# cvjena/mvlm

Hardware: AMD Instinct MI355X
Metric: views/sec (render+CNN+fuse) per mesh, 256x256x96 views (higher is better)
Workload: dtype f32; 1 GPU; configs[2] BU_3DFE-RGB+depth.json: 96 views @ 256x256 of one 99458-triangle textured synthetic face OBJ, 84 landmarks, 4 input channels (RGB+depth), seeded random weights; views_total=96, views_per_gpu=96, landmarks=84, in_channels=4, triangles=99458, selection_method=simple, parallelism=1 GPU, no collective

## Files before the change

mvlm_amd/csrc/conv_kernel.h:

```cpp
#ifndef MVLM_CONV_KERNEL_H
#define MVLM_CONV_KERNEL_H
#include <cstdlib>
#include <string>
#include <type_traits>

#include "common.h"

using f32x16 = __attribute__((ext_vector_type(16))) float;
using f32x4 = __attribute__((ext_vector_type(4))) float;

namespace {

constexpr unsigned INVALID_OFF = 0xFFFFFFFFu;

template <int I, int N, class F>
__device__ __forceinline__ void static_for(F&& f) {
    if constexpr (I < N) {
        f(std::integral_constant<int, I>{});
        static_for<I + 1, N>(f);
    }
}

template <int COUT_T_, int TW_, int TRI_, int NIMG_, int KS_, int CK_, bool SPLITK_ = false>
struct Cfg {
// ... 372 lines not shown
    const int e = tid + i * 256;
    return (e < C::WJOBS ? e : e - C::WJOBS) / ((C::TRI / 2) * C::PW);
}

template <class C>
__device__ __forceinline__ void wino_mask_tail(const ConvArgs& a, int cb, int tid, WinoStage<C>& ws) {
#pragma unroll
    for (int i = 0; i < C::X_ITERS; ++i) {
        const bool okc = cb + wino_job_channel<C>(tid, i) < a.cin;
#pragma unroll
        for (int q = 0; q < 3; ++q) ws.msk[i][q] = okc ? ws.msk[i][q] : 0u;
#pragma unroll
        for (int q = 0; q < 4; ++q) ws.off[i][q] = okc ? ws.off[i][q] : 0u;
    }
}

template <class C>
__device__ __forceinline__ void wino_main(const ConvArgs& a, float* smem, const int tid, const int y0, const int x0, const int b0,
                                          const int co0, const unsigned HWin, const int woff, f32x16 (&acc)[C::MT][C::NT], long long* t_loop) {
    static_assert(!C::WINO || (C::WT / 4) % 256 == 0, "every lane owns whole float4s of the weight slice");
    static_assert(!C::WINO || 256 * C::X_ITERS - C::WJOBS <= C::WJOBS, "a lane without a job repeats an earlier job");
    static_assert(!C::WINO || C::TRI % 2 == 0, "rows 2p and 2p + 1 of a tile share one mask: a tile is whole row pairs of an image whose height is a multiple of it");
    const int lane = tid & 63, wave = tid >> 6, half = lane >> 5, l31 = lane & 31;
    WinoStage<C> ws;
    constexpr int JPC = (C::TRI / 2) * C::PW;
#pragma unroll
    for (int i = 0; i < C::X_ITERS; ++i) {
        const int e0 = tid + i * 256;
        const int e = e0 < C::WJOBS ? e0 : e0 - C::WJOBS;
        const int c = e / JPC;
        const int rem = e - c * JPC;
        const int p = rem / C::PW;
        const int xx = rem - p * C::PW;
        const int y = y0 + 2 * p - 1, x = x0 + xx - 1;
        const bool okx = x >= 0 && x < a.W && b0 < a.B;
#pragma unroll
        for (int q = 0; q < 4; ++q) {
            const bool ok = okx && y + q >= 0 && y + q < a.H;
            ws.msk[i][q == 0 ? 0 : q == 3 ? 2 : 1] = ok ? 0xFFFFFFFFu : 0u;
            ws.off[i][q] = ok ? (unsigned(c) * HWin + unsigned((y + q) * a.W + x)) * 4u : 0u;
        }
        ws.lds[i] = c * C::PLANE + (p * C::PW + xx) * 4;
        ws.bn[i] = c;
    }
    {
        const int row = tid / (C::COUT_T / 4);
        const int c4 = tid - row * (C::COUT_T / 4);
        const int tap = row / C::CK;
        const int c = row - tap * C::CK;
        ws.woff = unsigned((tap * a.cin_pad + c) * a.cout_pad + co0 + c4 * 4) * 4u;
    }
    constexpr int TAPS_STEP = 256 / ((C::COUT_T / 4) * C::CK);
    static_assert(!C::WINO || 256 % ((C::COUT_T / 4) * C::CK) == 0, "256 float4s of the weight slice are whole taps");
    const size_t w_step = size_t(TAPS_STEP) * a.cin_pad * a.cout_pad * 4;
    ws.floor = __int_as_float(__builtin_amdgcn_readfirstlane(a.pre_scale != nullptr ? 0 : int(0xFF800000u)));
#pragma unroll
    for (int m = 0; m < C::MT; ++m) {
        ws.abase[m] = woff + m * 32;
        wino_opaque(ws.abase[m]);
    }
#pragma unroll
    for (int s = 0; s < 2; ++s)
#pragma unroll
        for (int cp = 0; cp < C::CK / 2; ++cp) {
            ws.bbase[s][cp] = s * C::STAGE + (2 * cp + half) * C::PLANE + (wave * C::WP * C::PW + l31) * 4;
            wino_opaque(ws.bbase[s][cp]);
        }
    float* const sbn = smem + 2 * C::STAGE;
    const char* const in0 = reinterpret_cast<const char*>(a.in + size_t((b0 < a.B ? b0 : 0) * a.in_ctot + a.in_coff) * HWin);
    const char* const w0 = reinterpret_cast<const char*>(a.w);
    constexpr int T_TOT = C::X_ITERS + C::W_ITERS;
    const int last = a.cin_pad - C::CK;
    const bool odd = (a.cin_pad / C::CK) & 1;
    if (last == 0) wino_mask_tail<C>(a, 0, tid, ws);
    static_for<0, T_TOT>([&](auto tc) { issue_item_wino<C, decltype(tc)::value>(in0, w0, w_step, ws); });
    for (int i = tid; i < a.cin_pad; i += 256) {
        sbn[2 * i] = a.pre_scale != nullptr ? a.pre_scale[i] : 1.f;
        sbn[2 * i + 1] = a.pre_scale != nullptr ? a.pre_shift[i] : -0.f;
    }
    __syncthreads();
    static_for<0, T_TOT>([&](auto tc) { bn_item_wino<C, decltype(tc)::value>(sbn, 0, ws); });
    if (odd) {
        static_for<0, T_TOT>([&](auto tc) { write_item_wino<C, decltype(tc)::value, 1>(smem, tid, ws); });
    } else {
        static_for<0, T_TOT>([&](auto tc) { write_item_wino<C, decltype(tc)::value, 0>(smem, tid, ws); });
    }
    __syncthreads();
#if defined(MVLM_CONV_TIMING)
    *t_loop = clock64();
#endif
    f32x16 wacc[C::MT][4 * C::WP];
#pragma unroll
    for (int m = 0; m < C::MT; ++m)
#pragma unroll
        for (int q = 0; q < 4 * C::WP; ++q) wacc[m][q] = f32x16{0.f, 0.f, 0.f, 0.f, 0.f, 0.f, 0.f, 0.f, 0.f, 0.f, 0.f, 0.f, 0.f, 0.f, 0.f, 0.f};
    if (last > 0) {
        int cb = 0;
        const size_t in_step = size_t(C::CK) * HWin * 4, w_cstep = size_t(C::CK) * a.cout_pad * 4;
        const char* in_nx = in0 + in_step;
        const char* w_nx = w0 + w_cstep;
        if (odd) {
            compute_chunk_wino<C, 1, true>(smem, sbn, in_nx, w_nx, w_step, C::CK, tid, ws, wacc);
            __syncthreads();
            cb = C::CK, in_nx += in_step, w_nx += w_cstep;
        }
        wino_forget_bases<C>(ws);
        for (; cb + C::CK < last; cb += 2 * C::CK) {
            compute_chunk_wino<C, 0, true>(smem, sbn, in_nx, w_nx, w_step, cb + C::CK, tid, ws, wacc);
            __syncthreads();
            in_nx += in_step, w_nx += w_cstep;
            compute_chunk_wino<C, 1, true>(smem, sbn, in_nx, w_nx, w_step, cb + 2 * C::CK, tid, ws, wacc);
            __syncthreads();
            in_nx += in_step, w_nx += w_cstep;
        }
        wino_forget_bases<C>(ws);
        wino_mask_tail<C>(a, last, tid, ws);
        compute_chunk_wino<C, 0, true>(smem, sbn, in_nx, w_nx, w_step, last, tid, ws, wacc);
        __syncthreads();
    }
    compute_chunk_wino<C, 1, false>(smem, sbn, nullptr, nullptr, 0, 0, tid, ws, wacc);
    static_for<0, C::MT>([&](auto mc) {
        constexpr int m = decltype(mc)::value;
        static_for<0, C::WP>([&](auto pc) {
            constexpr int p = decltype(pc)::value;
#pragma unroll
            for (int r = 0; r < 16; ++r) {
                const float m0 = wacc[m][4 * p][r], m1 = wacc[m][4 * p + 1][r], m2 = wacc[m][4 * p + 2][r], m3 = wacc[m][4 * p + 3][r];
                acc[m][2 * p][r] = (m0 + m1) + m2;
                acc[m][2 * p + 1][r] = (m1 - m2) - m3;
            }
        });
    });
    (void)t_loop;
}

template <class C>
struct Wino4Stage {
    static constexpr int N = C::WINO4 ? C::X_ITERS : 1;
    static constexpr int NW = C::WINO4 ? C::W_ITERS : 1;
    unsigned off[N][6];
    unsigned msk[N][3];
    int lds4[N], lds2[N];
    int bn[N];
    unsigned woff[NW];
    int wlds[NW];
    float xw[N][6];
    float bn_s[N], bn_t[N];
    f32x4 wv[NW];
    float floor;
    int abase;
    int bbase4[2][C::CK / 2], bbase2[2][C::CK / 2];
};

template <class C, int T>
__device__ __forceinline__ void issue_item_wino4(const char* in_cb, const char* w_cb, Wino4Stage<C>& ws) {
    if constexpr (T < C::X_ITERS) {
#pragma unroll
        for (int r = 0; r < 6; ++r) {
            wino_opaque(ws.off[T][r]);
            ws.xw[T][r] = *reinterpret_cast<const float*>(in_cb + ws.off[T][r]);
        }
    } else {
        constexpr int I = T - C::X_ITERS;
        wino_opaque(ws.woff[I]);
        ws.wv[I] = *reinterpret_cast<const f32x4*>(w_cb + ws.woff[I]);
    }
}

template <class C, int T>
__device__ __forceinline__ void bn_item_wino4(const float* sbn, int cb, Wino4Stage<C>& ws) {
    if constexpr (T < C::X_ITERS) {
        const float2 st = *reinterpret_cast<const float2*>(sbn + 2 * (cb + ws.bn[T]));
        ws.bn_s[T] = st.x;
        ws.bn_t[T] = st.y;
    }
}

template <class C, int T, int NEXT>
__device__ __forceinline__ void write_item_wino4(float* smem, const Wino4Stage<C>& ws) {
    if constexpr (T < C::X_ITERS) {
        float d[6];
#pragma unroll
        for (int r = 0; r < 6; ++r) {
            const float v = fmaxf(fmaf(ws.xw[T][r], ws.bn_s[T], ws.bn_t[T]), ws.floor);
            d[r] = __uint_as_float(__float_as_uint(v) & ws.msk[T][r == 0 ? 0 : r == 5 ? 2 : 1]);
        }
        const float v0 = fmaf(-1.5f, d[3], fmaf(-2.f, d[2], fmaf(1.5f, d[1], d[0]))) + d[4];
        const float v1 = fmaf(-0.5f, d[3], fmaf(-2.5f, d[2], -d[1])) + d[4];
        const float v2 = fmaf(-2.5f, d[3], fmaf(0.5f, d[2], d[1])) + d[4];
        const float v3 = fmaf(0.5f, d[3], fmaf(-0.5f, d[1], -d[2])) + d[4];
        const float v4 = fmaf(-2.f, d[3], fmaf(2.f, d[1], -d[2])) + d[4];
        const float v5 = fmaf(-1.5f, d[4], fmaf(-2.f, d[3], fmaf(1.5f, d[2], d[1]))) + d[5];
        *reinterpret_cast<f32x4*>(smem + NEXT * C::STAGE + ws.lds4[T]) = f32x4{v0, v1, v2, v3};
        *reinterpret_cast<float2*>(smem + NEXT * C::STAGE + ws.lds2[T]) = make_float2(v4, v5);
    } else {
        constexpr int I = T - C::X_ITERS;
        reinterpret_cast<f32x4*>(smem + NEXT * C::STAGE + C::XT_PAD)[ws.wlds[I]] = ws.wv[I];
    }
}

template <class C, int CUR, bool STAGE_NEXT>
__device__ __forceinline__ void compute_chunk_wino4(float* smem, const float* sbn, const char* in_cb, const char* w_cb, int cb_next,
                                                    Wino4Stage<C>& ws, f32x16 (&acc)[6]) {
    constexpr int T_TOT = C::X_ITERS + C::W_ITERS;
    constexpr int ISSUE_SPAN = C::KSTEPS / 2 > 0 ? C::KSTEPS / 2 : 1;
    constexpr int WRITE_SPAN = ISSUE_SPAN;
    constexpr int WRITE_START = C::KSTEPS - WRITE_SPAN;
    const float* const st = smem + CUR * C::STAGE;
    float av[2][6];
    f32x4 bv4[2];
    float2 bv2[2];
#pragma unroll
    for (int t = 0; t < 6; ++t) av[0][t] = st[ws.abase + t * 3 * C::CK * C::COUT_T];
    bv4[0] = *reinterpret_cast<const f32x4*>(smem + ws.bbase4[CUR][0]);
    bv2[0] = *reinterpret_cast<const float2*>(smem + ws.bbase2[CUR][0]);
    static_for<0, C::KSTEPS>([&](auto ksc) {
        constexpr int ks = decltype(ksc)::value;
        constexpr int nx = ks + 1;
        __builtin_amdgcn_s_waitcnt(0xC07F);
        __builtin_amdgcn_sched_barrier(0);
        if constexpr (nx < C::KSTEPS) {
            constexpr int kx = nx / (C::CK / 2), cp = nx % (C::CK / 2);
#pragma unroll
            for (int t = 0; t < 6; ++t) av[nx & 1][t] = st[ws.abase + ((t * 3 + kx) * C::CK + 2 * cp) * C::COUT_T];
            bv4[nx & 1] = *reinterpret_cast<const f32x4*>(smem + ws.bbase4[CUR][cp] + kx * 4);
            bv2[nx & 1] = *reinterpret_cast<const float2*>(smem + ws.bbase2[CUR][cp] + kx * 2);
        }
        auto bval = [&](auto tc) {
            constexpr int t = decltype(tc)::value;
            if constexpr (t < 4) return bv4[ks & 1][t];
            else if constexpr (t == 4) return bv2[ks & 1].x;
            else return bv2[ks & 1].y;
        };
        constexpr int LEAD = 2;
        static_for<0, 6>([&](auto tc) {
            constexpr int t = decltype(tc)::value;
            if constexpr (t < LEAD) acc[t] = __builtin_amdgcn_mfma_f32_32x32x2f32(av[ks & 1][t], bval(tc), acc[t], 0, 0, 0);
        });
        __builtin_amdgcn_sched_barrier(0);
        if constexpr (STAGE_NEXT) {
            if constexpr (ks >= WRITE_START) {
                constexpr int t_last = ((ks - WRITE_START + 1) * T_TOT + WRITE_SPAN - 1) / WRITE_SPAN - 1;
                static_assert(WRITE_START + (t_last * WRITE_SPAN) / T_TOT == ks && (t_last + 1 == T_TOT || WRITE_START + ((t_last + 1) * WRITE_SPAN) / T_TOT > ks));
                constexpr int later = (t_last + 1 < C::X_ITERS ? 6 * (C::X_ITERS - t_last - 1) + C::W_ITERS : T_TOT - t_last - 1);
                static_assert(later < 16);
                __builtin_amdgcn_s_waitcnt(0x0F70 | later);
                __builtin_amdgcn_sched_barrier(0);
            }
            static_for<0, T_TOT>([&](auto tc) {
                constexpr int t = decltype(tc)::value;
                if constexpr ((t * ISSUE_SPAN) / T_TOT == ks) {
                    issue_item_wino4<C, t>(in_cb, w_cb, ws);
                    bn_item_wino4<C, t>(sbn, cb_next, ws);
                }
                if constexpr (WRITE_START + (t * WRITE_SPAN) / T_TOT == ks) write_item_wino4<C, t, CUR ^ 1>(smem, ws);
            });
            __builtin_amdgcn_sched_barrier(0);
        }
        __builtin_amdgcn_s_setprio(1);
        static_for<0, 6>([&](auto tc) {
            constexpr int t = decltype(tc)::value;
            if constexpr (t >= LEAD) acc[t] = __builtin_amdgcn_mfma_f32_32x32x2f32(av[ks & 1][t], bval(tc), acc[t], 0, 0, 0);
        });
        __builtin_amdgcn_s_setprio(0);
        __builtin_amdgcn_sched_barrier(0);
    });
}

template <class C>
__device__ __forceinline__ void wino4_forget_bases(Wino4Stage<C>& ws) {
    wino_opaque(ws.abase);
#pragma unroll
    for (int s = 0; s < 2; ++s)
#pragma unroll
        for (int cp = 0; cp < C::CK / 2; ++cp) {
            wino_opaque(ws.bbase4[s][cp]);
            wino_opaque(ws.bbase2[s][cp]);
        }
#pragma unroll
    for (int i = 0; i < C::X_ITERS; ++i) {
        wino_opaque(ws.lds4[i]);
        wino_opaque(ws.lds2[i]);
    }
}

template <class C>
__device__ __forceinline__ int wino4_job_channel(int tid, int i) {
    const int e = tid + i * 256;
    return (e < C::WJOBS ? e : e - C::WJOBS) / ((C::TRI / 4) * C::PW);
}

template <class C>
__device__ __forceinline__ void wino4_mask_tail(const ConvArgs& a, int cb, int tid, Wino4Stage<C>& ws) {
#pragma unroll
    for (int i = 0; i < C::X_ITERS; ++i) {
        const bool okc = cb + wino4_job_channel<C>(tid, i) < a.cin;
#pragma unroll
        for (int q = 0; q < 3; ++q) ws.msk[i][q] = okc ? ws.msk[i][q] : 0u;
#pragma unroll
        for (int r = 0; r < 6; ++r) ws.off[i][r] = okc ? ws.off[i][r] : 0u;
    }
}

template <class C>
__device__ __forceinline__ void wino4_main(const ConvArgs& a, float* smem, const int tid, const int y0, const int x0, const int b0,
                                           const int co0, const unsigned HWin, const int woff, f32x16 (&acc)[C::EMT][C::ENT], long long* t_loop) {
    static_assert(!C::WINO4 || 256 * C::X_ITERS - C::WJOBS <= C::WJOBS, "a lane without a job repeats an earlier job");
    static_assert(!C::WINO4 || (C::TRI % 4 == 0 && C::ENT == 4 && C::EMT == 1), "one row quad per wave; rows 4q .. 4q + 3 of a tile share one mask");
    static_assert(!C::WINO4 || (C::WT / 4 > 256 * (C::W_ITERS - 1) && C::WT / 4 >= 256), "a lane without a float4 repeats its previous one");
    const int lane = tid & 63, wave = tid >> 6, half = lane >> 5, l31 = lane & 31;
    const int wq = C::WIDE4 ? (wave & 1) : wave;
    const int wh = C::WIDE4 ? (wave >> 1) : 0;
    Wino4Stage<C> ws;
    constexpr int JPC = (C::TRI / 4) * C::PW;
    constexpr int Q4 = JPC * 4;
#pragma unroll
    for (int i = 0; i < C::X_ITERS; ++i) {
        const int e0 = tid + i * 256;
        const int e = e0 < C::WJOBS ? e0 : e0 - C::WJOBS;
        const int c = e / JPC;
        const int rem = e - c * JPC;
        const int q = rem / C::PW;
        const int xx = rem - q * C::PW;
        const int y = y0 + 4 * q - 1, x = x0 + xx - 1;
        const bool okx = x >= 0 && x < a.W && b0 < a.B;
#pragma unroll
        for (int r = 0; r < 6; ++r) {
            const bool ok = okx && y + r >= 0 && y + r < a.H;
            if (r == 0 || r == 1 || r == 5) ws.msk[i][r == 0 ? 0 : r == 5 ? 2 : 1] = ok ? 0xFFFFFFFFu : 0u;
            ws.off[i][r] = ok ? (unsigned(c) * HWin + unsigned((y + r) * a.W + x)) * 4u : 0u;
        }
        ws.lds4[i] = c * C::PLANE + rem * 4;
        ws.lds2[i] = c * C::PLANE + Q4 + rem * 2;
        ws.bn[i] = c;
    }
#pragma unroll
    for (int i = 0; i < C::W_ITERS; ++i) {
        const int f0 = tid + i * 256;
        const int f = f0 < C::WT / 4 ? f0 : f0 - 256;
        const int row = f / (C::COUT_T / 4);
        const int c4 = f - row * (C::COUT_T / 4);
        const int tap = row / C::CK;
        const int c = row - tap * C::CK;
        ws.woff[i] = unsigned((tap * a.cin_pad + c) * a.cout_pad + co0 + c4 * 4) * 4u;
        ws.wlds[i] = f;
    }
    ws.floor = __int_as_float(__builtin_amdgcn_readfirstlane(a.pre_scale != nullptr ? 0 : int(0xFF800000u)));
    ws.abase = woff + 32 * wh;
    wino_opaque(ws.abase);
#pragma unroll
    for (int s = 0; s < 2; ++s)
#pragma unroll
        for (int cp = 0; cp < C::CK / 2; ++cp) {
            ws.bbase4[s][cp] = s * C::STAGE + (2 * cp + half) * C::PLANE + (wq * C::PW + l31) * 4;
            ws.bbase2[s][cp] = s * C::STAGE + (2 * cp + half) * C::PLANE + Q4 + (wq * C::PW + l31) * 2;
            wino_opaque(ws.bbase4[s][cp]);
            wino_opaque(ws.bbase2[s][cp]);
        }
    float* const sbn = smem + 2 * C::STAGE;
    const char* const in0 = reinterpret_cast<const char*>(a.in + size_t((b0 < a.B ? b0 : 0) * a.in_ctot + a.in_coff) * HWin);
    const char* const w0 = reinterpret_cast<const char*>(a.w);
    constexpr int T_TOT = C::X_ITERS + C::W_ITERS;
    const int last = a.cin_pad - C::CK;
    const bool odd = (a.cin_pad / C::CK) & 1;
    if (last == 0) wino4_mask_tail<C>(a, 0, tid, ws);
    static_for<0, T_TOT>([&](auto tc) { issue_item_wino4<C, decltype(tc)::value>(in0, w0, ws); });
    for (int i = tid; i < a.cin_pad; i += 256) {
        sbn[2 * i] = a.pre_scale != nullptr ? a.pre_scale[i] : 1.f;
        sbn[2 * i + 1] = a.pre_scale != nullptr ? a.pre_shift[i] : -0.f;
    }
    __syncthreads();
    static_for<0, T_TOT>([&](auto tc) { bn_item_wino4<C, decltype(tc)::value>(sbn, 0, ws); });
    if (odd) {
        static_for<0, T_TOT>([&](auto tc) { write_item_wino4<C, decltype(tc)::value, 1>(smem, ws); });
    } else {
        static_for<0, T_TOT>([&](auto tc) { write_item_wino4<C, decltype(tc)::value, 0>(smem, ws); });
    }
    __syncthreads();
#if defined(MVLM_CONV_TIMING)
    *t_loop = clock64();
#endif
    f32x16 wacc[6];
#pragma unroll
    for (int t = 0; t < 6; ++t) wacc[t] = f32x16{0.f, 0.f, 0.f, 0.f, 0.f, 0.f, 0.f, 0.f, 0.f, 0.f, 0.f, 0.f, 0.f, 0.f, 0.f, 0.f};
    if (last > 0) {
        int cb = 0;
        const size_t in_step = size_t(C::CK) * HWin * 4, w_cstep = size_t(C::CK) * a.cout_pad * 4;
        const char* in_nx = in0 + in_step;
        const char* w_nx = w0 + w_cstep;
        if (odd) {
            compute_chunk_wino4<C, 1, true>(smem, sbn, in_nx, w_nx, C::CK, ws, wacc);
            __syncthreads();
            cb = C::CK, in_nx += in_step, w_nx += w_cstep;
        }
        wino4_forget_bases<C>(ws);
        for (; cb + C::CK < last; cb += 2 * C::CK) {
            compute_chunk_wino4<C, 0, true>(smem, sbn, in_nx, w_nx, cb + C::CK, ws, wacc);
            __syncthreads();
            in_nx += in_step, w_nx += w_cstep;
            compute_chunk_wino4<C, 1, true>(smem, sbn, in_nx, w_nx, cb + 2 * C::CK, ws, wacc);
            __syncthreads();
            in_nx += in_step, w_nx += w_cstep;
        }
        wino4_forget_bases<C>(ws);
        wino4_mask_tail<C>(a, last, tid, ws);
        compute_chunk_wino4<C, 0, true>(smem, sbn, in_nx, w_nx, last, ws, wacc);
        __syncthreads();
    }
    compute_chunk_wino4<C, 1, false>(smem, sbn, nullptr, nullptr, 0, ws, wacc);
#pragma unroll
    for (int r = 0; r < 16; ++r) {
        const float m0 = wacc[0][r], m1 = wacc[1][r], m2 = wacc[2][r], m3 = wacc[3][r], m4 = wacc[4][r], m5 = wacc[5][r];
        const float s = m1 + m2, d = m1 - m2;
        acc[0][0][r] = (m0 + s) + (m3 + m4);
        acc[0][1][r] = d + fmaf(-0.5f, m4, 2.f * m3);
        acc[0][2][r] = s + fmaf(0.25f, m4, 4.f * m3);
        acc[0][3][r] = (d + fmaf(-0.125f, m4, 8.f * m3)) + m5;
    }
    (void)t_loop;
}

template <class C, bool AMAX, bool IN2 = false>
__device__ __forceinline__ void conv_tile(const ConvArgs& a_in, const int tiles_x, const int tiles_y, const int cout_tiles,
                                          const int bid, const int nblk) {
    extern __shared__ __attribute__((aligned(16))) float smem[];

    const int tid = threadIdx.x;
    const int lane = tid & 63;
    const int wave = tid >> 6;
    const int half = lane >> 5;
    const int l31 = lane & 31;

    int lid;
    {
        const int q = nblk >> 3, r = nblk & 7, xcd = bid & 7;
        lid = (xcd < r ? xcd * (q + 1) : r * (q + 1) + (xcd - r) * q) + (bid >> 3);
    }
    ConvArgs a_par;
    if constexpr (C::KS == 2) {
        a_par = a_in;
        if (a_in.n_par == 4) {
            const int pl = lid & 3;
            lid >>= 2;
            a_par.sub_y = pl >> 1;
            a_par.sub_x = pl & 1;
            a_par.w = a_in.w_par[pl];
            a_par.amax_part0 = a_in.amax_part0 + pl * a_in.amax_par_stride;
        }
    }
    const ConvArgs& a = C::KS == 2 ? a_par : a_in;
    int kp = 0;
    if constexpr (C::SPLITK) {
        if (a.kparts > 1) {
            kp = lid % a.kparts;
            lid /= a.kparts;
        }
    }
    const int tile_id = lid;
    const int ct = lid % cout_tiles;
    const int pt = lid / cout_tiles;
    const int tx = pt % tiles_x;
    const int ty = (pt / tiles_x) % tiles_y;
    const int tb = pt / (tiles_x * tiles_y);
    const int x0 = tx * C::TW, y0 = ty * C::TRI, b0 = tb * C::NIMG, co0 = ct * C::COUT_T;

#if defined(MVLM_CONV_TIMING)
    const long long t_start = clock64();
    long long t_loop = t_start;
#endif
    const int H = a.H, W = a.W;
    const int Hin = a.up_in ? (H >> 1) : H, Win = a.up_in ? (W >> 1) : W;
    const unsigned HWin = unsigned(Hin) * unsigned(Win);

    unsigned goff[C::X_ITERS];
    unsigned goff2[C::X_ITERS];
#pragma unroll
    for (int i = 0; i < C::X_ITERS; ++i) {
        const int e = tid + i * 256;
        const int c = e / C::PLANE;
        const int rem = e - c * C::PLANE;
        const int img = rem / (C::PH * C::PW);
        const int rem2 = rem - img * (C::PH * C::PW);
        const int yy = rem2 / C::PW;
        const int xx = rem2 - yy * C::PW;
        const int y = y0 + yy - C::HALO, x = x0 + xx - C::HALO, b = b0 + img;
        const bool ok = (e < C::XT) && y >= 0 && y < H && x >= 0 && x < W && b < a.B;
        const int ys = a.up_in ? (y >> 1) : y, xs = a.up_in ? (x >> 1) : x;
        goff[i] = ok ? (unsigned(b * a.in_ctot + a.in_coff + c) * HWin + unsigned(ys * Win + xs)) : INVALID_OFF;
        goff2[i] = (IN2 && ok) ? (unsigned(b * a.in2_ctot + c) * (HWin >> 2) + unsigned((ys >> 1) * (Win >> 1) + (xs >> 1))) : 0u;
    }
    unsigned woff_g[C::W_ITERS];
#pragma unroll
    for (int i = 0; i < C::W_ITERS; ++i) {
        const int f = tid + i * 256;
        const int row = f / (C::COUT_T / 4);
        const int c4 = f - row * (C::COUT_T / 4);
        const int tap = row / C::CK;
        const int c = row - tap * C::CK;
        woff_g[i] = (f < C::WT / 4) ? unsigned((tap * a.cin_pad + c) * a.cout_pad + co0 + c4 * 4) : INVALID_OFF;
    }

    int pixoff[C::NT];
#pragma unroll
    for (int n = 0; n < C::NT; ++n) {
        const int p = (C::SPLITK ? 0 : wave * (C::PIX_T / 4)) + n * 32 + l31;
        const int x = p % C::TW;
        const int rr = p / C::TW;
        const int yl = rr % C::TRI;
        const int img = rr / C::TRI;
        pixoff[n] = (img * C::PH + yl) * C::PW + x + half * C::PLANE + (C::KS == 2 ? a.sub_y * C::PW + a.sub_x : 0) +
                    (C::SPLITK ? wave * C::CKW * C::PLANE : 0);
    }
    const int woff = C::XT_PAD + half * C::COUT_T + l31 + (C::SPLITK ? wave * C::CKW * C::COUT_T : 0);

    f32x16 acc[C::EMT][C::ENT];
#pragma unroll
    for (int m = 0; m < C::EMT; ++m)
#pragma unroll
        for (int n = 0; n < C::ENT; ++n) acc[m][n] = f32x16{0.f, 0.f, 0.f, 0.f, 0.f, 0.f, 0.f, 0.f, 0.f, 0.f, 0.f, 0.f, 0.f, 0.f, 0.f, 0.f};
    const int q16 = lane >> 4, i16 = lane & 15;
    const int woff16 = C::XT_PAD + q16 * C::COUT_T + C::MT * 32 + i16;
    int pixoff16[C::NT16];
    f32x4 acc16[C::NT16];
#pragma unroll
    for (int j = 0; j < C::NT16; ++j) {
        const int p = wave * (C::PIX_T / 4) + j * 16 + i16;
        pixoff16[j] = (p / C::TW % C::TRI) * C::PW + p % C::TW + q16 * C::PLANE + (C::KS == 2 ? a.sub_y * C::PW + a.sub_x : 0);
        acc16[j] = f32x4{0.f, 0.f, 0.f, 0.f};
    }

    Strip4 s4;
    if constexpr (C::TAIL4) {
        const int p = wave * (C::PIX_T / 4) + lane;
        s4.woff4 = C::XT_PAD + C::MT * 32 + 16 + (lane & 3);
        s4.pixoff4 = (p / C::TW % C::TRI) * C::PW + p % C::TW + (C::KS == 2 ? a.sub_y * C::PW + a.sub_x : 0);
    }
    float* sbn = smem + 2 * C::STAGE;
    StageRegs<C> regs;
    constexpr int T_TOT = C::X_ITERS + C::W_ITERS;
    int cb0 = 0, cb1 = a.cin_pad;
    if constexpr (C::SPLITK) {
        const int span = a.cin_pad / a.kparts;
        cb0 = kp * span;
        cb1 = cb0 + span;
    }
    SplitKTails<C::SPLITK ? C::NT : 1> sks;
    if constexpr (C::SPLITK) {
        if (a.kparts <= 1) {
#pragma unroll
            for (int n = 0; n < C::NT; ++n) {
                SplitKTail& sk = sks.t[n];
                const int p = n * 32 + l31;
                const int rr = p / C::TW;
                const int b = b0 + rr / C::TRI;
                const int y = y0 + rr % C::TRI, x = x0 + p % C::TW;
                sk.ok = C::NIMG == 1 ? true : (b < a.B);
                sk.b = sk.ok ? unsigned(b) : 0u;
                sk.pix = unsigned(y * a.W + x);
                sk.y = y;
                sk.x = x;
                const unsigned HWo = unsigned(a.H) * unsigned(a.W);
                const int cl = co0 + 8 * wave + 4 * half;
// ... 683 lines not shown
    if constexpr (C::TAIL16) {
        const unsigned b = unsigned(b0);
#pragma unroll
        for (int j = 0; j < C::NT16; ++j) {
            const int p = wave * (C::PIX_T / 4) + j * 16 + i16;
            const int y = y0 + p / C::TW, x = x0 + p % C::TW;
            pix16[j] = a.up_out == 2 ? (2 * y + a.sub_y) * (2 * W) + 2 * x + a.sub_x : y * W + x;
        }
        const unsigned plane = a.up_out == 2 ? 4u * HW : HW;
#pragma unroll
        for (int i = 0; i < 4; ++i) {
            const int co = co0 + C::MT * 32 + 4 * q16 + i;
            ok16[i] = co < a.cout;
            const int coc = ok16[i] ? co : 0;
            const float bias = a.bias ? a.bias[coc] : 0.f;
            float* const po = a.out ? a.out + (size_t(b) * a.out_ctot + a.out_coff + coc) * plane : nullptr;
#pragma unroll
            for (int j = 0; j < C::NT16; ++j) {
                val16[j][i] = acc16[j][i] + bias;
                if (po && ok16[i]) po[pix16[j]] = val16[j][i];
            }
        }
    }
    if constexpr (C::TAIL4) {
        const int p = wave * (C::PIX_T / 4) + lane;
        const int y = y0 + p / C::TW, x = x0 + p % C::TW;
        const unsigned pix = a.up_out == 2 ? unsigned(2 * y + a.sub_y) * unsigned(2 * W) + unsigned(2 * x + a.sub_x)
                                           : unsigned(y) * unsigned(W) + unsigned(x);
        const unsigned plane = a.up_out == 2 ? 4u * HW : HW;
#pragma unroll
        for (int v = 0; v < 4; ++v) {
            const int co = co0 + C::MT * 32 + 16 + v;
            if (co < a.cout && a.out)
                a.out[(size_t(b0) * a.out_ctot + a.out_coff + co) * plane + pix] = s4.acc[v] + (a.bias ? a.bias[co] : 0.f);
        }
    }

}

template <class C, bool AMAX, bool IN2 = false>
__global__ __launch_bounds__(256, C::MIN_BLOCKS_PER_CU) void conv_mfma_kernel(const ConvArgs a_in, const int tiles_x, const int tiles_y,
                                                           const int cout_tiles) {
    conv_tile<C, AMAX, IN2>(a_in, tiles_x, tiles_y, cout_tiles, int(blockIdx.x), int(gridDim.x));
}

struct ConvPairArgs {
    ConvArgs a[2];
    int tiles_x[2], tiles_y[2], cout_tiles[2], nblk[2];
    int nblk0_pad;
};

template <class C>
__global__ __launch_bounds__(256, C::MIN_BLOCKS_PER_CU) void conv_pair_kernel(const ConvPairArgs p) {
    const int bid = int(blockIdx.x);
    const int which = bid >= p.nblk0_pad ? 1 : 0;
    if (!which && bid >= p.nblk[0]) return;
    conv_tile<C, false>(p.a[which], p.tiles_x[which], p.tiles_y[which], p.cout_tiles[which], which ? bid - p.nblk0_pad : bid,
                        p.nblk[which]);
}

struct ConvGrid {
    int tiles_x = 0, tiles_y = 0, cout_tiles = 0;
    long tiles = 0;
    long nblk = 0;
};

template <class C>
int check_variant(mvlm_ctx* ctx, ConvArgs& a, ConvGrid& g) {
    const int tiles_x = a.W / C::TW, tiles_y = a.H / C::TRI;
    const int tiles_b = (a.B + C::NIMG - 1) / C::NIMG;
    const int cout_tiles = a.cout_pad / C::COUT_T;
    MVLM_REQUIRE(ctx, a.ksize == C::KS, "conv: kernel variant built for another kernel size");
    MVLM_REQUIRE(ctx, !a.in2 || (C::HAS_IN2 && !a.up_in && !a.amax_val && a.in_coff == 0 && a.in2_ctot >= a.cin && !(a.H & 1) && !(a.W & 1) && a.kparts <= 1),
                 "conv: a second input tensor (upsample + skip on the load) is served by the 128-channel 8x32 tile only");
    MVLM_REQUIRE(ctx, !C::WINO || (!a.up_in && !a.in2 && !a.amax_val && a.up_out != 2 && a.n_par == 1 && a.kparts <= 1),
                 "conv: the Winograd tiles serve plain, pooling and scattering 3x3 layers (no upsampled / second input, no fused argmax, no K parts)");
    MVLM_REQUIRE(ctx, !C::WINO4 || (!a.up_in && !a.in2 && !a.amax_val && a.up_out != 2 && a.n_par == 1 && a.kparts <= 1),
                 "conv: the F(4,3) Winograd tile serves plain, pooling and scattering 3x3 layers (no upsampled / second input, no fused argmax, no K parts)");
    MVLM_REQUIRE(ctx, a.W % C::TW == 0 && a.H % C::TRI == 0, "conv: spatial size not a multiple of the tile");
    MVLM_REQUIRE(ctx, !C::SPLITK || a.cin_pad % 32 == 0, "conv: split-K tiles need 32-channel chunks");
    MVLM_REQUIRE(ctx, !(C::SPLITK && C::NT > 1) || (a.kparts <= 1 && !a.amax_val), "conv: the two-column split-K tiles have no K-parts / argmax form");
    MVLM_REQUIRE(ctx, a.cout_pad % C::COUT_T == 0, "conv: cout_pad not a multiple of the cout tile");
    MVLM_REQUIRE(ctx, a.cin_pad % C::CK == 0, "conv: cin_pad must be a multiple of the K-chunk");
    MVLM_REQUIRE(ctx, !a.pre_scale || a.cin_pad <= C::BN_MAXC, "conv: pre-activation BatchNorm supports up to 256 input channels");
    MVLM_REQUIRE(ctx, !C::WINO || a.cin_pad <= C::BN_MAXC, "conv: the Winograd tiles keep a BatchNorm pair of every input channel in LDS, with or without pre-activation (up to 256)");
    MVLM_REQUIRE(ctx, !C::WINO4 || a.cin_pad <= C::BN_MAXC, "conv: the F(4,3) Winograd tile keeps a BatchNorm pair of every input channel in LDS, with or without pre-activation (up to 256)");
    if (C::TAIL4) MVLM_REQUIRE(ctx, a.up_out != 1 && (a.out || (a.amax_val && C::HAS_AMAX)), "conv: the 84-channel tile writes a plain (or parity) output tensor or argmax partials");
    if (C::TAIL16)
        MVLM_REQUIRE(ctx, !a.res1 && !a.res2 && !a.out_raw && !a.post_scale && a.up_out != 1 && !a.pool_out,
                     "conv: the 80-channel tiles serve plain conv + bias layers only");
    if (a.amax_val) {
        MVLM_REQUIRE(ctx, C::NIMG == 1, "conv: fused argmax needs one image per tile");
        MVLM_REQUIRE(ctx, a.amax_part0 >= 0 && a.amax_part0 + tiles_x * tiles_y * 4 <= a.amax_parts,
                     "conv: argmax partial range mismatch");
        MVLM_REQUIRE(ctx, !a.res1 && !a.post_scale && a.up_out != 1, "conv: fused argmax expects a plain conv + bias layer");
        MVLM_REQUIRE(ctx, !a.out && !a.out_raw && !a.pool_out, "conv: a fused-argmax launch does not materialise the heatmap");
    }
    long nblk = long(tiles_x) * tiles_y * tiles_b * cout_tiles;
    if (a.n_par != 1) {
        MVLM_REQUIRE(ctx, a.n_par == 4 && C::KS == 2 && a.up_out == 2, "conv: four parities per launch are a 2x2-kernel feature");
        MVLM_REQUIRE(ctx, a.w_par[0] && a.w_par[1] && a.w_par[2] && a.w_par[3], "conv: parity weights missing");
        MVLM_REQUIRE(ctx, !a.amax_val || (a.amax_par_stride >= tiles_x * tiles_y * 4 &&
                                          a.amax_part0 + 3 * a.amax_par_stride + tiles_x * tiles_y * 4 <= a.amax_parts),
                     "conv: argmax partial range mismatch (four parities)");
        nblk *= 4;
    }
    MVLM_REQUIRE(ctx, nblk > 0 && nblk < (1l << 31), "conv: bad grid");
    a.kparts = a.kparts > 1 ? a.kparts : 1;
    g.tiles = nblk;
    if (a.kparts > 1) {
        MVLM_REQUIRE(ctx, C::SPLITK, "conv: only the split-K tiles divide the input channels over workgroups");
        MVLM_REQUIRE(ctx, a.cin_pad % (a.kparts * C::CK) == 0, "conv: input channels do not divide into the requested K parts");
        nblk *= a.kparts;
    }
    MVLM_REQUIRE(ctx, nblk < (1l << 31), "conv: bad grid");
    g.tiles_x = tiles_x;
    g.tiles_y = tiles_y;
    g.cout_tiles = cout_tiles;
    g.nblk = nblk;
    return 0;
}

template <class C>
int set_variant_attributes(mvlm_ctx* ctx, int attr_bit) {
    if ((ctx->conv_attr_mask >> attr_bit) & 1ull) return 0;
    MVLM_CHECK_HIP(ctx, hipFuncSetAttribute(reinterpret_cast<const void*>(conv_mfma_kernel<C, false>),
                                            hipFuncAttributeMaxDynamicSharedMemorySize, int(C::LDS_BYTES)));
    if constexpr (C::HAS_AMAX)
        MVLM_CHECK_HIP(ctx, hipFuncSetAttribute(reinterpret_cast<const void*>(conv_mfma_kernel<C, true>),
                                                hipFuncAttributeMaxDynamicSharedMemorySize, int(C::LDS_BYTES)));
    if constexpr (C::PAIRABLE)
        MVLM_CHECK_HIP(ctx, hipFuncSetAttribute(reinterpret_cast<const void*>(conv_pair_kernel<C>),
                                                hipFuncAttributeMaxDynamicSharedMemorySize, int(C::LDS_BYTES)));
    if constexpr (C::HAS_IN2)
        MVLM_CHECK_HIP(ctx, hipFuncSetAttribute(reinterpret_cast<const void*>(conv_mfma_kernel<C, false, true>),
                                                hipFuncAttributeMaxDynamicSharedMemorySize, int(C::LDS_BYTES)));
    ctx->conv_attr_mask |= 1ull << attr_bit;
    return 0;
}

template <class C>
int launch_variant(mvlm_ctx* ctx, const ConvArgs& a_in, int attr_bit) {
    ConvArgs a = a_in;
#if defined(MVLM_CONV_TIMING)
    if (const char* e = getenv("MVLM_CONV_TIMING_BUF")) a.timing = reinterpret_cast<unsigned long long*>(strtoull(e, nullptr, 0));
#endif
    ConvGrid g;
    if (check_variant<C>(ctx, a, g)) return 1;
    if (a.kparts > 1) {
        MVLM_REQUIRE(ctx, g.tiles <= MVLM_KPARTS_MAX_TILES && g.nblk <= MVLM_KPARTS_MAX_PARTS, "conv: too many tiles for the K-part workspace");
        if (mvlm_conv_kparts_workspace(ctx, &a.kws, &a.kcnt)) return 1;
    }
    if (set_variant_attributes<C>(ctx, attr_bit)) return 1;
    if (a.amax_val) {
        if constexpr (C::HAS_AMAX) {
            hipLaunchKernelGGL((conv_mfma_kernel<C, true>), dim3((unsigned)g.nblk), dim3(256), C::LDS_BYTES, ctx->cur_stream(),
                               a, g.tiles_x, g.tiles_y, g.cout_tiles);
        } else {
            return ctx->fail("conv: fused argmax is only built for the 8x32-pixel tile variants");
        }
    } else if (a.in2) {
        if constexpr (C::HAS_IN2) {
            hipLaunchKernelGGL((conv_mfma_kernel<C, false, true>), dim3((unsigned)g.nblk), dim3(256), C::LDS_BYTES, ctx->cur_stream(), a,
                               g.tiles_x, g.tiles_y, g.cout_tiles);
        } else {
            return ctx->fail("conv: this kernel variant has no second-input form");
        }
    } else {
        hipLaunchKernelGGL((conv_mfma_kernel<C, false>), dim3((unsigned)g.nblk), dim3(256), C::LDS_BYTES, ctx->cur_stream(), a,
                           g.tiles_x, g.tiles_y, g.cout_tiles);
    }
    MVLM_CHECK_HIP(ctx, hipGetLastError());
    return 0;
}

template <class C>
int launch_variant_pair(mvlm_ctx* ctx, const ConvArgs& a0, const ConvArgs& a1, int attr_bit) {
    if constexpr (!C::PAIRABLE) {
        return ctx->fail("conv: this kernel variant has no two-problem form");
    } else {
        ConvPairArgs p;
        p.a[0] = a0;
        p.a[1] = a1;
        ConvGrid g[2];
        for (int i = 0; i < 2; ++i) {
            ConvArgs& a = p.a[i];
            MVLM_REQUIRE(ctx, !a.amax_val && a.n_par == 1 && !a.timing && !a.in2, "conv: a paired launch takes plain convolutions");
            if (check_variant<C>(ctx, a, g[i])) return 1;
        }
        if (p.a[0].kparts > 1 || p.a[1].kparts > 1) {
            const long t0 = p.a[0].kparts > 1 ? g[0].tiles : 0, n0 = p.a[0].kparts > 1 ? g[0].nblk : 0;
            const long t1 = p.a[1].kparts > 1 ? g[1].tiles : 0, n1 = p.a[1].kparts > 1 ? g[1].nblk : 0;
            MVLM_REQUIRE(ctx, t0 + t1 <= MVLM_KPARTS_MAX_TILES && n0 + n1 <= MVLM_KPARTS_MAX_PARTS, "conv: too many tiles for the K-part workspace");
            float* kws = nullptr;
            unsigned* kcnt = nullptr;
            if (mvlm_conv_kparts_workspace(ctx, &kws, &kcnt)) return 1;
            p.a[0].kws = kws;
            p.a[0].kcnt = kcnt;
            p.a[1].kws = kws + size_t(n0) * 1024;
            p.a[1].kcnt = kcnt + t0;
        }
        for (int i = 0; i < 2; ++i) {
            p.tiles_x[i] = g[i].tiles_x;
            p.tiles_y[i] = g[i].tiles_y;
            p.cout_tiles[i] = g[i].cout_tiles;
            p.nblk[i] = int(g[i].nblk);
        }
        p.nblk0_pad = (p.nblk[0] + 7) / 8 * 8;
        const long total = long(p.nblk0_pad) + p.nblk[1];
        MVLM_REQUIRE(ctx, total < (1l << 31), "conv: bad grid");
        if (set_variant_attributes<C>(ctx, attr_bit)) return 1;
        hipLaunchKernelGGL((conv_pair_kernel<C>), dim3((unsigned)total), dim3(256), C::LDS_BYTES, ctx->cur_stream(), p);
        MVLM_CHECK_HIP(ctx, hipGetLastError());
        return 0;
    }
}


}
#endif
```

Baseline: 1344 views/s.

## Interleave Winograd staging loads and writes between individual MFMAs in each k-step

Replaces the coarse per-k-step staging schedule in the Winograd F(4,3) conv path with a compile-time plan. The plan splits each input tile's global loads, BN fetch and transform/LDS write into small slices and places one slice group after every MFMA, so memory and VALU work is spread evenly across the matrix-core stream. The pointer advance and BN offset increment move inside the chunk, and the setprio/LEAD split is removed. A timing-only hook to launch with inflated LDS (to limit occupancy) is also added under MVLM_CONV_TIMING. Finer interleaving needs more precise waitcnt accounting and may raise register pressure.

```diff
diff --git a/mvlm_amd/csrc/conv_kernel.h b/mvlm_amd/csrc/conv_kernel.h
--- a/mvlm_amd/csrc/conv_kernel.h
+++ b/mvlm_amd/csrc/conv_kernel.h
@@ -548,13 +548,51 @@
     int bbase4[2][C::CK / 2], bbase2[2][C::CK / 2];
 };
 
-template <class C, int T>
-__device__ __forceinline__ void issue_item_wino4(const char* in_cb, const char* w_cb, Wino4Stage<C>& ws) {
+template <class C>
+struct Wino4Plan {
+    static constexpr int NX = C::WINO4 ? C::X_ITERS : 1, NW = C::WINO4 ? C::W_ITERS : 1;
+    static constexpr int GAPS = 6 * C::KSTEPS;
+    static constexpr int XI = 4, XW = 6;
+    static constexpr int NI = XI * NX + NW, NWR = XW * NX + NW;
+    static constexpr int ADVANCE = 6 * (C::KSTEPS / 2) - 1;
+    static constexpr int wfirst(int i) { return i * NW / NX; }
+    static constexpr int slices(int t, int per) { return t < NX ? per : 1; }
+    static constexpr int seq(int t, int p, int per) {
+        if (t < NX) return t * per + wfirst(t) + p;
+        int i = 0;
+        while (wfirst(i + 1) <= t - NX) ++i;
+        return (i + 1) * per + (t - NX);
+    }
+    static constexpr int issue_gap(int t, int p) { return (seq(t, p, XI) / 5) * 6 + seq(t, p, XI) % 5; }
+    static constexpr int write_gap(int t, int p) { return GAPS - 1 - NWR + seq(t, p, XW); }
+    static constexpr int loads(int t, int p) { return t >= NX ? 1 : p < 3 ? 2 : 0; }
+    static constexpr int later(int t) {
+        int n = 0;
+        for (int u = 0; u < NX + NW; ++u)
+            for (int q = 0; q < slices(u, XI); ++q)
+                if (seq(u, q, XI) > seq(t, slices(t, XI) - 1, XI) && issue_gap(u, q) <= write_gap(t, 0)) n += loads(u, q);
+        return n;
+    }
+    static constexpr bool ordered() {
+        for (int t = 0; t < NX + NW; ++t)
+            if (issue_gap(t, slices(t, XI) - 1) >= write_gap(t, 0) || issue_gap(t, slices(t, XI) - 1) > ADVANCE || later(t) >= 16) return false;
+        return true;
+    }
+};
+
+template <class C, int T, int P>
+__device__ __forceinline__ void issue_slice_wino4(const char* in_cb, const char* w_cb, const float* sbn, Wino4Stage<C>& ws) {
     if constexpr (T < C::X_ITERS) {
-#pragma unroll
-        for (int r = 0; r < 6; ++r) {
-            wino_opaque(ws.off[T][r]);
-            ws.xw[T][r] = *reinterpret_cast<const float*>(in_cb + ws.off[T][r]);
+        if constexpr (P < 3) {
+#pragma unroll
+            for (int r = 2 * P; r < 2 * P + 2; ++r) {
+                wino_opaque(ws.off[T][r]);
+                ws.xw[T][r] = *reinterpret_cast<const float*>(in_cb + ws.off[T][r]);
+            }
+        } else {
+            const float2 st = *reinterpret_cast<const float2*>(sbn + 2 * ws.bn[T]);
+            ws.bn_s[T] = st.x;
+            ws.bn_t[T] = st.y;
         }
     } else {
         constexpr int I = T - C::X_ITERS;
@@ -564,48 +602,97 @@
 }
 
 template <class C, int T>
-__device__ __forceinline__ void bn_item_wino4(const float* sbn, int cb, Wino4Stage<C>& ws) {
+__device__ __forceinline__ void issue_item_wino4(const char* in_cb, const char* w_cb, Wino4Stage<C>& ws) {
     if constexpr (T < C::X_ITERS) {
-        const float2 st = *reinterpret_cast<const float2*>(sbn + 2 * (cb + ws.bn[T]));
-        ws.bn_s[T] = st.x;
-        ws.bn_t[T] = st.y;
-    }
-}
-
-template <class C, int T, int NEXT>
-__device__ __forceinline__ void write_item_wino4(float* smem, const Wino4Stage<C>& ws) {
+        static_for<0, 3>([&](auto pc) { issue_slice_wino4<C, T, decltype(pc)::value>(in_cb, w_cb, nullptr, ws); });
+    } else {
+        issue_slice_wino4<C, T, 0>(in_cb, w_cb, nullptr, ws);
+    }
+}
+
+template <class C, int T>
+__device__ __forceinline__ void bn_item_wino4(const float* sbn, Wino4Stage<C>& ws) {
+    if constexpr (T < C::X_ITERS) issue_slice_wino4<C, T, 3>(nullptr, nullptr, sbn, ws);
+}
+
+template <class C, int T, int P, int NEXT>
+__device__ __forceinline__ void write_slice_wino4(float* smem, Wino4Stage<C>& ws, float (&v01)[2]) {
     if constexpr (T < C::X_ITERS) {
-        float d[6];
-#pragma unroll
-        for (int r = 0; r < 6; ++r) {
-            const float v = fmaxf(fmaf(ws.xw[T][r], ws.bn_s[T], ws.bn_t[T]), ws.floor);
-            d[r] = __uint_as_float(__float_as_uint(v) & ws.msk[T][r == 0 ? 0 : r == 5 ? 2 : 1]);
-        }
-        const float v0 = fmaf(-1.5f, d[3], fmaf(-2.f, d[2], fmaf(1.5f, d[1], d[0]))) + d[4];
-        const float v1 = fmaf(-0.5f, d[3], fmaf(-2.5f, d[2], -d[1])) + d[4];
-        const float v2 = fmaf(-2.5f, d[3], fmaf(0.5f, d[2], d[1])) + d[4];
-        const float v3 = fmaf(0.5f, d[3], fmaf(-0.5f, d[1], -d[2])) + d[4];
-        const float v4 = fmaf(-2.f, d[3], fmaf(2.f, d[1], -d[2])) + d[4];
-        const float v5 = fmaf(-1.5f, d[4], fmaf(-2.f, d[3], fmaf(1.5f, d[2], d[1]))) + d[5];
-        *reinterpret_cast<f32x4*>(smem + NEXT * C::STAGE + ws.lds4[T]) = f32x4{v0, v1, v2, v3};
-        *reinterpret_cast<float2*>(smem + NEXT * C::STAGE + ws.lds2[T]) = make_float2(v4, v5);
+        float(&d)[6] = ws.xw[T];
+        if constexpr (P < 3) {
+#pragma unroll
+            for (int r = 2 * P; r < 2 * P + 2; ++r) {
+                const float v = fmaxf(fmaf(d[r], ws.bn_s[T], ws.bn_t[T]), ws.floor);
+                d[r] = __uint_as_float(__float_as_uint(v) & ws.msk[T][r == 0 ? 0 : r == 5 ? 2 : 1]);
+            }
+        } else if constexpr (P == 3) {
+            v01[0] = fmaf(-1.5f, d[3], fmaf(-2.f, d[2], fmaf(1.5f, d[1], d[0]))) + d[4];
+            v01[1] = fmaf(-0.5f, d[3], fmaf(-2.5f, d[2], -d[1])) + d[4];
+        } else if constexpr (P == 4) {
+            const float v2 = fmaf(-2.5f, d[3], fmaf(0.5f, d[2], d[1])) + d[4];
+            const float v3 = fmaf(0.5f, d[3], fmaf(-0.5f, d[1], -d[2])) + d[4];
+            *reinterpret_cast<f32x4*>(smem + NEXT * C::STAGE + ws.lds4[T]) = f32x4{v01[0], v01[1], v2, v3};
+        } else {
+            const float v4 = fmaf(-2.f, d[3], fmaf(2.f, d[1], -d[2])) + d[4];
+            const float v5 = fmaf(-1.5f, d[4], fmaf(-2.f, d[3], fmaf(1.5f, d[2], d[1]))) + d[5];
+            *reinterpret_cast<float2*>(smem + NEXT * C::STAGE + ws.lds2[T]) = make_float2(v4, v5);
+        }
     } else {
         constexpr int I = T - C::X_ITERS;
         reinterpret_cast<f32x4*>(smem + NEXT * C::STAGE + C::XT_PAD)[ws.wlds[I]] = ws.wv[I];
     }
 }
 
+template <class C, int T, int NEXT>
+__device__ __forceinline__ void write_item_wino4(float* smem, Wino4Stage<C>& ws) {
+    float v01[2];
+    static_for<0, Wino4Plan<C>::slices(T, Wino4Plan<C>::XW)>([&](auto pc) { write_slice_wino4<C, T, decltype(pc)::value, NEXT>(smem, ws, v01); });
+}
+
+template <class C>
+__device__ __forceinline__ void wino4_advance(const char*& in_cb, const char*& w_cb, size_t in_step, size_t w_step, Wino4Stage<C>& ws) {
+    in_cb += in_step, w_cb += w_step;
+#pragma unroll
+    for (int i = 0; i < C::X_ITERS; ++i) ws.bn[i] += C::CK;
+}
+
+template <class C, int G, int NEXT>
+__device__ __forceinline__ void gap_wino4(float* smem, const float* sbn, const char*& in_cb, const char*& w_cb, size_t in_step, size_t w_step,
+                                          Wino4Stage<C>& ws, float (&v01)[2]) {
+    using P = Wino4Plan<C>;
+    static_for<0, P::NX + P::NW>([&](auto tc) {
+        constexpr int t = decltype(tc)::value;
+        static_for<0, P::slices(t, P::XI)>([&](auto pc) {
+            constexpr int p = decltype(pc)::value;
+            if constexpr (P::issue_gap(t, p) == G) issue_slice_wino4<C, t, p>(in_cb, w_cb, sbn, ws);
+        });
+    });
+    static_for<0, P::NX + P::NW>([&](auto tc) {
+        constexpr int t = decltype(tc)::value;
+        static_for<0, P::slices(t, P::XW)>([&](auto pc) {
+            constexpr int p = decltype(pc)::value;
+            if constexpr (P::write_gap(t, p) == G) {
+                if constexpr (p == 0) {
+                    __builtin_amdgcn_s_waitcnt(0x0F70 | P::later(t));
+                    __builtin_amdgcn_sched_barrier(0);
+                }
+                write_slice_wino4<C, t, p, NEXT>(smem, ws, v01);
+            }
+        });
+    });
+    if constexpr (G == P::ADVANCE) wino4_advance<C>(in_cb, w_cb, in_step, w_step, ws);
+}
+
 template <class C, int CUR, bool STAGE_NEXT>
-__device__ __forceinline__ void compute_chunk_wino4(float* smem, const float* sbn, const char* in_cb, const char* w_cb, int cb_next,
-                                                    Wino4Stage<C>& ws, f32x16 (&acc)[6]) {
-    constexpr int T_TOT = C::X_ITERS + C::W_ITERS;
-    constexpr int ISSUE_SPAN = C::KSTEPS / 2 > 0 ? C::KSTEPS / 2 : 1;
-    constexpr int WRITE_SPAN = ISSUE_SPAN;
-    constexpr int WRITE_START = C::KSTEPS - WRITE_SPAN;
+__device__ __forceinline__ void compute_chunk_wino4(float* smem, const float* sbn, const char*& in_cb, const char*& w_cb, size_t in_step,
+                                                    size_t w_step, Wino4Stage<C>& ws, f32x16 (&acc)[6]) {
+    using P = Wino4Plan<C>;
+    static_assert(P::NI <= 5 * (C::KSTEPS / 2) && P::NWR <= P::GAPS - 1 && P::ordered(), "loads in the first half of the k-steps, every write behind its loads");
     const float* const st = smem + CUR * C::STAGE;
     float av[2][6];
     f32x4 bv4[2];
     float2 bv2[2];
+    float v01[2];
 #pragma unroll
     for (int t = 0; t < 6; ++t) av[0][t] = st[ws.abase + t * 3 * C::CK * C::COUT_T];
     bv4[0] = *reinterpret_cast<const f32x4*>(smem + ws.bbase4[CUR][0]);
@@ -628,38 +715,15 @@
             else if constexpr (t == 4) return bv2[ks & 1].x;
             else return bv2[ks & 1].y;
         };
-        constexpr int LEAD = 2;
         static_for<0, 6>([&](auto tc) {
             constexpr int t = decltype(tc)::value;
-            if constexpr (t < LEAD) acc[t] = __builtin_amdgcn_mfma_f32_32x32x2f32(av[ks & 1][t], bval(tc), acc[t], 0, 0, 0);
+            acc[t] = __builtin_amdgcn_mfma_f32_32x32x2f32(av[ks & 1][t], bval(tc), acc[t], 0, 0, 0);
+            __builtin_amdgcn_sched_barrier(0);
+            if constexpr (STAGE_NEXT) {
+                gap_wino4<C, 6 * ks + t, CUR ^ 1>(smem, sbn, in_cb, w_cb, in_step, w_step, ws, v01);
+                __builtin_amdgcn_sched_barrier(0);
+            }
         });
-        __builtin_amdgcn_sched_barrier(0);
-        if constexpr (STAGE_NEXT) {
-            if constexpr (ks >= WRITE_START) {
-                constexpr int t_last = ((ks - WRITE_START + 1) * T_TOT + WRITE_SPAN - 1) / WRITE_SPAN - 1;
-                static_assert(WRITE_START + (t_last * WRITE_SPAN) / T_TOT == ks && (t_last + 1 == T_TOT || WRITE_START + ((t_last + 1) * WRITE_SPAN) / T_TOT > ks));
-                constexpr int later = (t_last + 1 < C::X_ITERS ? 6 * (C::X_ITERS - t_last - 1) + C::W_ITERS : T_TOT - t_last - 1);
-                static_assert(later < 16);
-                __builtin_amdgcn_s_waitcnt(0x0F70 | later);
-                __builtin_amdgcn_sched_barrier(0);
-            }
-            static_for<0, T_TOT>([&](auto tc) {
-                constexpr int t = decltype(tc)::value;
-                if constexpr ((t * ISSUE_SPAN) / T_TOT == ks) {
-                    issue_item_wino4<C, t>(in_cb, w_cb, ws);
-                    bn_item_wino4<C, t>(sbn, cb_next, ws);
-                }
-                if constexpr (WRITE_START + (t * WRITE_SPAN) / T_TOT == ks) write_item_wino4<C, t, CUR ^ 1>(smem, ws);
-            });
-            __builtin_amdgcn_sched_barrier(0);
-        }
-        __builtin_amdgcn_s_setprio(1);
-        static_for<0, 6>([&](auto tc) {
-            constexpr int t = decltype(tc)::value;
-            if constexpr (t >= LEAD) acc[t] = __builtin_amdgcn_mfma_f32_32x32x2f32(av[ks & 1][t], bval(tc), acc[t], 0, 0, 0);
-        });
-        __builtin_amdgcn_s_setprio(0);
-        __builtin_amdgcn_sched_barrier(0);
     });
 }
 
@@ -766,7 +830,7 @@
         sbn[2 * i + 1] = a.pre_scale != nullptr ? a.pre_shift[i] : -0.f;
     }
     __syncthreads();
-    static_for<0, T_TOT>([&](auto tc) { bn_item_wino4<C, decltype(tc)::value>(sbn, 0, ws); });
+    static_for<0, T_TOT>([&](auto tc) { bn_item_wino4<C, decltype(tc)::value>(sbn, ws); });
     if (odd) {
         static_for<0, T_TOT>([&](auto tc) { write_item_wino4<C, decltype(tc)::value, 1>(smem, ws); });
     } else {
@@ -782,28 +846,28 @@
     if (last > 0) {
         int cb = 0;
         const size_t in_step = size_t(C::CK) * HWin * 4, w_cstep = size_t(C::CK) * a.cout_pad * 4;
-        const char* in_nx = in0 + in_step;
-        const char* w_nx = w0 + w_cstep;
+        const char* in_nx = in0;
+        const char* w_nx = w0;
+        wino4_advance<C>(in_nx, w_nx, in_step, w_cstep, ws);
         if (odd) {
-            compute_chunk_wino4<C, 1, true>(smem, sbn, in_nx, w_nx, C::CK, ws, wacc);
+            compute_chunk_wino4<C, 1, true>(smem, sbn, in_nx, w_nx, in_step, w_cstep, ws, wacc);
             __syncthreads();
-            cb = C::CK, in_nx += in_step, w_nx += w_cstep;
+            cb = C::CK;
         }
         wino4_forget_bases<C>(ws);
         for (; cb + C::CK < last; cb += 2 * C::CK) {
-            compute_chunk_wino4<C, 0, true>(smem, sbn, in_nx, w_nx, cb + C::CK, ws, wacc);
+            compute_chunk_wino4<C, 0, true>(smem, sbn, in_nx, w_nx, in_step, w_cstep, ws, wacc);
             __syncthreads();
-            in_nx += in_step, w_nx += w_cstep;
-            compute_chunk_wino4<C, 1, true>(smem, sbn, in_nx, w_nx, cb + 2 * C::CK, ws, wacc);
+            compute_chunk_wino4<C, 1, true>(smem, sbn, in_nx, w_nx, in_step, w_cstep, ws, wacc);
             __syncthreads();
-            in_nx += in_step, w_nx += w_cstep;
         }
         wino4_forget_bases<C>(ws);
         wino4_mask_tail<C>(a, last, tid, ws);
-        compute_chunk_wino4<C, 0, true>(smem, sbn, in_nx, w_nx, last, ws, wacc);
+        compute_chunk_wino4<C, 0, true>(smem, sbn, in_nx, w_nx, in_step, w_cstep, ws, wacc);
         __syncthreads();
     }
-    compute_chunk_wino4<C, 1, false>(smem, sbn, nullptr, nullptr, 0, ws, wacc);
+    const char* none = nullptr;
+    compute_chunk_wino4<C, 1, false>(smem, sbn, none, none, 0, 0, ws, wacc);
 #pragma unroll
     for (int r = 0; r < 16; ++r) {
         const float m0 = wacc[0][r], m1 = wacc[1][r], m2 = wacc[2][r], m3 = wacc[3][r], m4 = wacc[4][r], m5 = wacc[5][r];
@@ -1793,6 +1857,22 @@
         if (mvlm_conv_kparts_workspace(ctx, &a.kws, &a.kcnt)) return 1;
     }
     if (set_variant_attributes<C>(ctx, attr_bit)) return 1;
+#if defined(MVLM_CONV_TIMING)
+    if constexpr (C::WINO4) {
+        if (const char* e = getenv("MVLM_CONV_TIMING_WINO4_LDS")) {
+            const size_t lds = strtoull(e, nullptr, 0);
+            if (lds > size_t(C::LDS_BYTES) && !a.amax_val && !a.in2) {
+                MVLM_REQUIRE(ctx, lds <= 160 * 1024, "conv: MVLM_CONV_TIMING_WINO4_LDS beyond a CU's LDS");
+                MVLM_CHECK_HIP(ctx, hipFuncSetAttribute(reinterpret_cast<const void*>(conv_mfma_kernel<C, false>),
+                                                        hipFuncAttributeMaxDynamicSharedMemorySize, int(lds)));
+                hipLaunchKernelGGL((conv_mfma_kernel<C, false>), dim3((unsigned)g.nblk), dim3(256), lds, ctx->cur_stream(), a,
+                                   g.tiles_x, g.tiles_y, g.cout_tiles);
+                MVLM_CHECK_HIP(ctx, hipGetLastError());
+                return 0;
+            }
+        }
+    }
+#endif
     if (a.amax_val) {
         if constexpr (C::HAS_AMAX) {
             hipLaunchKernelGGL((conv_mfma_kernel<C, true>), dim3((unsigned)g.nblk), dim3(256), C::LDS_BYTES, ctx->cur_stream(),
```

Result: faster. 1380 views/s (median of 6 runs) (+2.7%).
